# autonomousvision/gaussian-opacity-fields

Hardware: NVIDIA H100
Metric: training views/sec (fwd+bwd) @1080p, 1M Gaussians (higher is better)
Workload: dtype f32

## Files before the change

### gaussian-opacity-fields_b200/csrc/api.cu

```cuda
#include <stdarg.h>
#include <stdlib.h>

#include <chrono>

#include "gof_common.cuh"

static bool gof_trace_on() {
  static int on = -1;
  if (on < 0) { const char* e = getenv("GOF_TRACE"); on = (e && e[0] == '1') ? 1 : 0; }
  return on == 1;
}
struct GofTrace {
  std::chrono::steady_clock::time_point t0 = std::chrono::steady_clock::now();
  double last = 0;
  void mark(const char* what) {
    if (!gof_trace_on()) return;
    double t = std::chrono::duration<double, std::micro>(std::chrono::steady_clock::now() - t0).count();
    fprintf(stderr, "[gof trace] %-22s +%9.1f us (t=%9.1f us)\n", what, t - last, t);
    last = t;
  }
};

#include <map>
#include <mutex>
// ... 106 lines not shown
  static thread_local SideCopy table[64];
  int dev = 0;
  if (cudaGetDevice(&dev) != cudaSuccess || dev < 0 || dev >= 64) return nullptr;
  SideCopy& s = table[dev];
  if (!s.tried) {
    s.tried = true;
    s.ok = cudaStreamCreateWithFlags(&s.st, cudaStreamNonBlocking) == cudaSuccess &&
           cudaEventCreateWithFlags(&s.after_kernel, cudaEventDisableTiming) == cudaSuccess &&
           cudaEventCreateWithFlags(&s.copied, cudaEventDisableTiming) == cudaSuccess &&
           cudaHostAlloc((void**)&s.pin, 64, cudaHostAllocDefault) == cudaSuccess;
    if (!s.ok) (void)cudaGetLastError();
  }
  return s.ok ? &s : nullptr;
}
}

static SideCopy* begin_async_read_u32(const void* src_dev, cudaStream_t st) {
  SideCopy* sc = side_copy_for_current_device();
  if (!sc) return nullptr;
  if (cudaEventRecord(sc->after_kernel, st) != cudaSuccess || cudaStreamWaitEvent(sc->st, sc->after_kernel, 0) != cudaSuccess ||
      cudaMemcpyAsync(sc->pin, src_dev, 4, cudaMemcpyDeviceToHost, sc->st) != cudaSuccess ||
      cudaEventRecord(sc->copied, sc->st) != cudaSuccess) {
    (void)cudaGetLastError();
    return nullptr;
  }
  return sc;
}
static int finish_async_read_u32(SideCopy* sc, uint32_t* out) {
  GOF_CUDA_OK(cudaEventSynchronize(sc->copied));
  *out = *sc->pin;
  return GOF_OK;
}

static int preprocess_sort_count(const gof_scene_t* s, const GofView& v, char* geom, const GofGeomLayout& GL, int* radii,
                                 float box_margin, cudaStream_t st, uint32_t* R) {
  int rc;
  if ((rc = gof_launch_preprocess(s, v, geom, GL, radii, box_margin, st)) != GOF_OK) return rc;
  SideCopy* sc = s->debug ? nullptr : begin_async_read_u32(geom + GL.total, st);
  if ((rc = gof_depth_sort(s->P, geom, GL, s->debug != 0, st)) != GOF_OK) return rc;
  if (sc) return finish_async_read_u32(sc, R);
  return gof_read_back(R, geom + GL.total, sizeof(uint32_t), st);
}

static unsigned long long* g_stats_dev = nullptr;
unsigned long long* gof_stats_buffer() {
  static int on = -1;
  if (on < 0) { const char* e = getenv("GOF_STATS"); on = (e && e[0] == '1') ? 1 : 0; }
  if (!on) return nullptr;
  if (!g_stats_dev) { cudaMalloc(&g_stats_dev, 8 * sizeof(unsigned long long)); cudaMemset(g_stats_dev, 0, 8 * sizeof(unsigned long long)); }
  return g_stats_dev;
}
extern "C" int gof_stats_read(unsigned long long* out) {
  if (!gof_stats_buffer()) return 0;
  cudaMemcpy(out, g_stats_dev, 8 * sizeof(unsigned long long), cudaMemcpyDeviceToHost);
  cudaMemset(g_stats_dev, 0, 8 * sizeof(unsigned long long));
  return 1;
}

static thread_local char g_err[1024] = "";

void gof_set_error(const char* fmt, ...) {
  va_list ap;
  va_start(ap, fmt);
  vsnprintf(g_err, sizeof(g_err), fmt, ap);
  va_end(ap);
}

extern "C" const char* gof_last_error(void) { return g_err; }
extern "C" int gof_version(void) { return 100; }

// ... 25 lines not shown
  if (!has_sr && !s->view2gaussian_precomp) {
    gof_set_error("scales/rotations absent: view2gaussian_precomp is required");
    return GOF_E_INVALID;
  }
  if (s->width > 16 * 65535 || s->height > 16 * 65535) { gof_set_error("image too large"); return GOF_E_INVALID; }
  return GOF_OK;
}

extern "C" int gof_rasterize_forward(const gof_scene_t* s, gof_alloc_fn geom_alloc, void* geom_user,
                                     gof_alloc_fn binning_alloc, void* binning_user, gof_alloc_fn image_alloc,
                                     void* image_user, float* out_color, int* radii, int* num_rendered,
                                     void* stream) {
  int rc = validate_scene(s);
  if (rc != GOF_OK) return rc;
  if (!geom_alloc || !binning_alloc || !image_alloc || !num_rendered) {
    gof_set_error("allocators / num_rendered must be non-NULL");
    return GOF_E_INVALID;
  }
  *num_rendered = 0;
  cudaStream_t st = (cudaStream_t)stream;
  if (s->P == 0) return GOF_OK;
  if (!out_color || !radii) { gof_set_error("out_color / radii must be non-NULL"); return GOF_E_INVALID; }
  const GofView v = gof_make_view(s);

  GofTrace tr;
  const GofGeomLayout GL = gof_geom_layout((size_t)s->P);
  char* geom = (char*)geom_alloc(geom_user, GL.bytes);
  const GofImageLayout IL = gof_image_layout(s->width, s->height);
  char* img = (char*)image_alloc(image_user, IL.bytes);
  if (!geom || !img) { gof_set_error("scratch allocator returned NULL"); return GOF_E_ALLOC; }
  tr.mark("alloc geom+img");

  uint32_t R = 0;
  if ((rc = preprocess_sort_count(s, v, geom, GL, radii, 0.0f, st, &R)) != GOF_OK) return rc;
  *num_rendered = (int)R;
  tr.mark("pre+sort, num_rendered");

  const GofBinLayout BL = gof_bin_layout((size_t)R, s->width, s->height);
  char* bin = (char*)binning_alloc(binning_user, BL.bytes);
  if (!bin && BL.bytes) { gof_set_error("binning allocator returned NULL"); return GOF_E_ALLOC; }
  tr.mark("alloc binning");

  if ((rc = gof_bin_tiles(s->P, (size_t)R, v, geom, GL, bin, BL, img, IL, s->debug != 0, st)) != GOF_OK) return rc;
  if ((rc = gof_launch_render_forward(s, v, geom, GL, bin, BL, img, IL, out_color, st)) != GOF_OK) return rc;
  tr.mark("launch bin+render");
  return GOF_OK;
}

extern "C" int gof_rasterize_backward(const gof_scene_t* s, int num_rendered, const int* radii,
                                      void* geom_buffer, const void* binning_buffer,
                                      const void* image_buffer, const float* dL_dpix, float* dL_dmean2D,
                                      float* dL_dconic, float* dL_dopacity, float* dL_dcolor, float* dL_dmean3D,
                                      float* dL_dcov3D, float* dL_dsh, float* dL_dscale, float* dL_drot,
                                      float* dL_dview2gaussian, void* stream) {
  return gof_rasterize_backward_stats(s, num_rendered, radii, geom_buffer, binning_buffer, image_buffer, dL_dpix, dL_dmean2D, dL_dconic,
                                      dL_dopacity, dL_dcolor, dL_dmean3D, dL_dcov3D, dL_dsh, dL_dscale, dL_drot, dL_dview2gaussian,
                                      nullptr, nullptr, stream);
}

extern "C" int gof_rasterize_backward_stats(const gof_scene_t* s, int num_rendered, const int* radii, void* geom_buffer,
                                            const void* binning_buffer, const void* image_buffer, const float* dL_dpix,
                                            float* dL_dmean2D, float* dL_dconic, float* dL_dopacity, float* dL_dcolor,
                                            float* dL_dmean3D, float* dL_dcov3D, float* dL_dsh, float* dL_dscale, float* dL_drot,
                                            float* dL_dview2gaussian, float* dens_sum, float* dens_max, void* stream) {
  return gof_rasterize_backward_dp(s, num_rendered, radii, geom_buffer, binning_buffer, image_buffer, dL_dpix, dL_dmean2D, dL_dconic,
                                   dL_dopacity, dL_dcolor, dL_dmean3D, dL_dcov3D, dL_dsh, dL_dscale, dL_drot, dL_dview2gaussian, dens_sum,
                                   dens_max, nullptr, nullptr, stream);
// ... 247 lines not shown
```

### gaussian-opacity-fields_b200/csrc/binning.cu

```cuda
#include "gof_common.cuh"

namespace {

constexpr int THREADS = GOF_BLOCK_SIZE;
constexpr int WARPS = THREADS / 32;
constexpr uint32_t LB_AGG = 1u << 30;
constexpr uint32_t LB_INC = 2u << 30;
constexpr uint32_t LB_VAL = (1u << 30) - 1u;
constexpr size_t LB_MAX_ITEMS = (size_t)1 << 30;

__device__ __forceinline__ uint32_t ld_volatile(const uint32_t* p) { return *reinterpret_cast<const volatile uint32_t*>(p); }
__device__ __forceinline__ void st_volatile(uint32_t* p, uint32_t v) { *reinterpret_cast<volatile uint32_t*>(p) = v; }
__device__ __forceinline__ uint64_t ld_volatile(const uint64_t* p) { return *reinterpret_cast<const volatile uint64_t*>(p); }
__device__ __forceinline__ void st_volatile(uint64_t* p, uint64_t v) { *reinterpret_cast<volatile uint64_t*>(p) = v; }

template <typename W> struct LbWord;
template <> struct LbWord<uint32_t> {
  static constexpr int SHIFT = 30;
  static constexpr uint32_t VAL = LB_VAL;
};
template <> struct LbWord<uint64_t> {
  static constexpr int SHIFT = 32;
  static constexpr uint64_t VAL = 0xffffffffull;
};
// ... 35 lines not shown
}
__device__ __forceinline__ uint32_t lookback_digit_walk(uint32_t* status, uint32_t digit, uint32_t chunk, uint32_t aggregate) {
  uint32_t* own = status + ((size_t)(chunk >> 2) * GOF_RADIX + digit) * 4 + (chunk & 3u);
  if (chunk == 0) return 0u;
  uint32_t excl = 0u;
  uint32_t pos = chunk;
  while (pos > 0) {
    const uint32_t g = (pos - 1u) >> 2;
    const uint32_t need = pos - 4u * g;
    const uint32_t* word = status + ((size_t)g * GOF_RADIX + digit) * 4;
    uint4 w;
    bool ready;
    do {
      w = ld_volatile_v4(word);
      ready = (w.x >> 30) != 0u && (need < 2u || (w.y >> 30) != 0u) && (need < 3u || (w.z >> 30) != 0u) && (need < 4u || (w.w >> 30) != 0u);
    } while (!ready);
    const uint32_t e[4] = {w.x, w.y, w.z, w.w};
    bool done = false;
#pragma unroll
    for (int i = 3; i >= 0; --i) {
      if (!done && (uint32_t)i < need) {
        excl += e[i] & LB_VAL;
        if ((e[i] >> 30) == 2u) done = true;
      }
    }
    if (done) break;
    pos = 4u * g;
  }
  st_volatile(own, LB_INC | (excl + aggregate));
  return excl;
}

struct Digits { int shift[4]; uint32_t mask[4]; int passes; };

template <typename KeyT>
__global__ void __launch_bounds__(THREADS) k_digit_hist(const KeyT* __restrict__ keys, size_t n, Digits dg, uint32_t* __restrict__ ghist) {
  __shared__ uint32_t s_h[4][GOF_RADIX];
#pragma unroll
  for (int p = 0; p < 4; ++p) s_h[p][threadIdx.x] = 0;
  __syncthreads();
  const size_t stride = (size_t)gridDim.x * THREADS;
  for (size_t i = (size_t)blockIdx.x * THREADS + threadIdx.x; i < n; i += stride) {
    const uint32_t k = (uint32_t)keys[i];
#pragma unroll
    for (int p = 0; p < 4; ++p)
      if (p < dg.passes) atomicAdd(&s_h[p][(k >> dg.shift[p]) & dg.mask[p]], 1u);
  }
  __syncthreads();
#pragma unroll
  for (int p = 0; p < 4; ++p)
    if (p < dg.passes && s_h[p][threadIdx.x]) atomicAdd(ghist + p * GOF_RADIX + threadIdx.x, s_h[p][threadIdx.x]);
}

template <typename KeyT>
__global__ void __launch_bounds__(THREADS, 3) k_onesweep(const KeyT* __restrict__ keys_in, const uint32_t* __restrict__ vals_in,
                                                        KeyT* __restrict__ keys_out, uint32_t* __restrict__ vals_out, size_t n,
                                                        int shift, uint32_t mask, const uint32_t* __restrict__ ghist,
                                                        uint32_t* __restrict__ status ,
                                                        uint32_t* __restrict__ ticket) {
  __shared__ uint32_t s_cnt[WARPS][GOF_RADIX];
  __shared__ uint32_t s_gbase[GOF_RADIX];
  __shared__ uint32_t s_lbase[GOF_RADIX];
  __shared__ KeyT s_keys[GOF_SORT_CHUNK];
  __shared__ uint32_t s_vals[GOF_SORT_CHUNK];
  __shared__ uint32_t s_chunk;
  const int lane = threadIdx.x & 31, warp = threadIdx.x >> 5;
  if (threadIdx.x == 0) s_chunk = atomicAdd(ticket, 1u);
#pragma unroll
  for (int w = 0; w < WARPS; ++w) s_cnt[w][threadIdx.x] = 0;
  uint32_t dig_total;
  const uint32_t gstart = block_excl_scan(threadIdx.x <= mask ? ghist[threadIdx.x] : 0u, &dig_total);
  const uint32_t chunk = s_chunk;
  const size_t cbase = (size_t)chunk * GOF_SORT_CHUNK;
  const size_t wbase = cbase + (size_t)warp * (GOF_SORT_ITEMS * 32);

  KeyT key[GOF_SORT_ITEMS];
  uint32_t rank[GOF_SORT_ITEMS];
#pragma unroll
  for (int r = 0; r < GOF_SORT_ITEMS; ++r) {
    const size_t i = wbase + (size_t)r * 32 + lane;
    key[r] = i < n ? keys_in[i] : (KeyT)0;
  }
  const uint32_t lt = (1u << lane) - 1u;
#pragma unroll
  for (int r = 0; r < GOF_SORT_ITEMS; ++r) {
    const size_t i = wbase + (size_t)r * 32 + lane;
    const bool valid = i < n;
    const uint32_t d = valid ? (((uint32_t)key[r] >> shift) & mask) : (uint32_t)GOF_RADIX;
    const uint32_t peers = __match_any_sync(0xffffffffu, d);
    const int leader = __ffs(peers) - 1;
    uint32_t old = 0;
    if (lane == leader && valid) {
      old = s_cnt[warp][d];
      s_cnt[warp][d] = old + __popc(peers);
    }
    old = __shfl_sync(0xffffffffu, old, leader);
    rank[r] = old + __popc(peers & lt);
    __syncwarp();
  }
  __syncthreads();
  uint32_t count = 0;
  if (threadIdx.x <= mask) {
#pragma unroll
    for (int w = 0; w < WARPS; ++w) {
      const uint32_t c = s_cnt[w][threadIdx.x];
      s_cnt[w][threadIdx.x] = count;
      count += c;
    }
    lookback_digit_publish(status, threadIdx.x, chunk, count);
  }
  uint32_t chunk_n;
  const uint32_t lstart = block_excl_scan(count, &chunk_n);
  s_lbase[threadIdx.x] = lstart;
  __syncthreads();
#pragma unroll
  for (int r = 0; r < GOF_SORT_ITEMS; ++r) {
    const size_t i = wbase + (size_t)r * 32 + lane;
    if (i < n) {
      const uint32_t d = ((uint32_t)key[r] >> shift) & mask;
      const uint32_t lp = s_lbase[d] + s_cnt[warp][d] + rank[r];
      s_keys[lp] = key[r];
      s_vals[lp] = vals_in[i];
    }
  }
  if (threadIdx.x <= mask) s_gbase[threadIdx.x] = gstart + lookback_digit_walk(status, threadIdx.x, chunk, count);
  __syncthreads();
#pragma unroll
  for (int r = 0; r < GOF_SORT_ITEMS; ++r) {
    const uint32_t i = (uint32_t)r * THREADS + threadIdx.x;
    if (i < chunk_n) {
      const KeyT k = s_keys[i];
      const uint32_t d = ((uint32_t)k >> shift) & mask;
      const uint32_t pos = s_gbase[d] + (i - s_lbase[d]);
      keys_out[pos] = k;
      vals_out[pos] = s_vals[i];
    }
  }
}

struct SortScratch {
  uint32_t* ghist;
  uint32_t* tickets;
  uint32_t* status;
  size_t pass_words;
};

SortScratch carve_sort_scratch(uint32_t* scratch, size_t n) {
  SortScratch s;
  s.ghist = scratch;
  s.tickets = scratch + 4 * GOF_RADIX;
  s.status = scratch + GOF_SORT_HEAD_BYTES / 4;
  s.pass_words = (size_t)((gof_sort_blocks(n) + 3) / 4 + 1) * GOF_RADIX * 4;
  return s;
}

void split_digits(int nbits, Digits* dg) {
  dg->passes = (nbits + 7) / 8;
  int rem = nbits, shift = 0;
  for (int p = 0; p < 4; ++p) { dg->shift[p] = 0; dg->mask[p] = 0; }
  for (int p = 0; p < dg->passes; ++p) {
    const int b = (rem + (dg->passes - p) - 1) / (dg->passes - p);
    dg->shift[p] = shift; dg->mask[p] = (1u << b) - 1u;
    shift += b; rem -= b;
  }
}

template <typename KeyT>
int onesweep_passes(KeyT* ka, KeyT* kb, uint32_t* va, uint32_t* vb, size_t n, const Digits& dg, const SortScratch& sc, bool debug,
                    cudaStream_t st) {
  const unsigned nb = (unsigned)gof_sort_blocks(n);
  for (int p = 0; p < dg.passes; ++p) {
    const bool a2b = (p % 2 == 0);
    GOF_LAUNCH("radix_onesweep", st, (k_onesweep<KeyT><<<nb, THREADS, 0, st>>>(
        a2b ? ka : kb, a2b ? va : vb, a2b ? kb : ka, a2b ? vb : va, n, dg.shift[p], dg.mask[p], sc.ghist + p * GOF_RADIX,
        sc.status + (size_t)p * sc.pass_words, sc.tickets + p)));
    GOF_LAUNCH_CHECK(debug, st);
  }
  return GOF_OK;
}

int sm_count() {
  static int sms = 0;
  if (!sms) { int dev = 0; cudaGetDevice(&dev); cudaDeviceGetAttribute(&sms, cudaDevAttrMultiProcessorCount, dev); if (sms <= 0) sms = 132; }
  return sms;
}

template <typename KeyT>
int sort_pairs(KeyT* ka, KeyT* kb, uint32_t* va, uint32_t* vb, uint32_t* scratch, size_t n, int nbits, bool debug, cudaStream_t st,
               int* result_in_b) {
  *result_in_b = 0;
  if (n == 0 || nbits <= 0) return GOF_OK;
  if (n >= LB_MAX_ITEMS) { gof_set_error("radix sort of %zu items: fewer than 2^30 supported", n); return GOF_E_INVALID; }
  Digits dg;
  split_digits(nbits, &dg);
  const SortScratch sc = carve_sort_scratch(scratch, n);
  GOF_CUDA_OK(cudaMemsetAsync(scratch, 0, GOF_SORT_HEAD_BYTES + (size_t)dg.passes * sc.pass_words * 4, st));
  const size_t want = (n + (size_t)THREADS * 8 - 1) / ((size_t)THREADS * 8);
  const unsigned grid = (unsigned)(want < (size_t)sm_count() * 4 ? want : (size_t)sm_count() * 4);
  GOF_LAUNCH("radix_hist", st, k_digit_hist<KeyT><<<grid, THREADS, 0, st>>>(ka, n, dg, sc.ghist));
  GOF_LAUNCH_CHECK(debug, st);
  const int rc = onesweep_passes<KeyT>(ka, kb, va, vb, n, dg, sc, debug, st);
  *result_in_b = dg.passes % 2;
  return rc;
}

__global__ void __launch_bounds__(THREADS) k_scan_excl(const uint32_t* __restrict__ in, uint32_t* __restrict__ out, size_t n,
                                                      uint64_t* __restrict__ status, uint32_t* __restrict__ ticket,
                                                      uint32_t* __restrict__ total_out, uint32_t nchunks) {
  __shared__ uint32_t s_chunk, s_prefix;
  if (threadIdx.x == 0) s_chunk = atomicAdd(ticket, 1u);
  __syncthreads();
  const uint32_t chunk = s_chunk;
  const size_t base = (size_t)chunk * GOF_SCAN_CHUNK + (size_t)threadIdx.x * GOF_SCAN_ITEMS;
  uint32_t v[GOF_SCAN_ITEMS];
  uint32_t s = 0;
#pragma unroll
  for (int k = 0; k < GOF_SCAN_ITEMS; ++k) {
    v[k] = (base + k < n) ? in[base + k] : 0u;
    s += v[k];
  }
  uint32_t total;
  uint32_t run = block_excl_scan(s, &total);
  if (threadIdx.x < 32) {
    const uint32_t excl = lookback_warp(status, chunk, total);
    if (threadIdx.x == 0) {
      s_prefix = excl;
      if (chunk == nchunks - 1 && total_out) *total_out = excl + total;
    }
  }
  __syncthreads();
  run += s_prefix;
#pragma unroll
  for (int k = 0; k < GOF_SCAN_ITEMS; ++k) {
    if (base + k < n) out[base + k] = run;
    run += v[k];
  }
}

template <typename KeyT>
__global__ void __launch_bounds__(THREADS) k_scan_emit(int P, const uint32_t* __restrict__ order, const uint2* __restrict__ rect,
                                                      const uint32_t* __restrict__ tiles, int grid_x, KeyT* __restrict__ keys,
                                                      uint32_t* __restrict__ vals, uint32_t* __restrict__ status,
                                                      uint32_t* __restrict__ ticket, Digits dg, uint32_t* __restrict__ ghist,
                                                      uint32_t capacity) {
  __shared__ uint32_t s_off[THREADS + 1];
  __shared__ uint32_t s_g[THREADS];
  __shared__ uint2 s_rect[THREADS];
  __shared__ uint32_t s_h[2][GOF_RADIX];
  __shared__ uint32_t s_chunk, s_prefix;
  if (threadIdx.x == 0) s_chunk = atomicAdd(ticket, 1u);
  s_h[0][threadIdx.x] = 0; s_h[1][threadIdx.x] = 0;
  __syncthreads();
  const uint32_t chunk = s_chunk;
  const int k = (int)(chunk * THREADS + threadIdx.x);
  uint32_t g = 0, n = 0;
  uint2 rc = make_uint2(0u, 0u);
  if (k < P) {
    g = order[k];
    n = tiles[g];
    if (n) rc = rect[g];
  }
  uint32_t total;
  const uint32_t lo = block_excl_scan(n, &total);
  s_off[threadIdx.x] = lo; s_g[threadIdx.x] = g; s_rect[threadIdx.x] = rc;
  if (threadIdx.x < 32) {
    const uint32_t excl = lookback_warp(status, chunk, total);
    if (threadIdx.x == 0) { s_off[THREADS] = total; s_prefix = excl; }
  }
  __syncthreads();
  const uint32_t prefix = s_prefix;
  for (uint32_t j = threadIdx.x; j < total; j += THREADS) {
    int lo_i = 0, hi_i = THREADS;
    while (hi_i - lo_i > 1) {
      const int mid = (lo_i + hi_i) >> 1;
      if (s_off[mid] <= j) lo_i = mid; else hi_i = mid;
    }
    const uint32_t t = j - s_off[lo_i];
    const uint2 r = s_rect[lo_i];
    const uint32_t xmin = r.x & 0xffffu, ymin = r.x >> 16;
    const uint32_t w = (r.y & 0xffffu) - xmin;
    const uint32_t dy = t / w, dx = t - dy * w;
    const uint32_t tile = (ymin + dy) * (uint32_t)grid_x + xmin + dx;
    const uint32_t pos = prefix + j;
    if (pos < capacity) {
      keys[pos] = (KeyT)tile;
      vals[pos] = s_g[lo_i];
    }
    atomicAdd(&s_h[0][(tile >> dg.shift[0]) & dg.mask[0]], 1u);
    if (dg.passes > 1) atomicAdd(&s_h[1][(tile >> dg.shift[1]) & dg.mask[1]], 1u);
  }
// ... 16 lines not shown
      ranges[cur].x = (uint32_t)idx;
    }
  }
  if (idx == L - 1) ranges[cur].y = (uint32_t)L;
}

template <typename KeyT>
int bin_tiles_t(int P, size_t R, const GofView& v, char* geom, const GofGeomLayout& GL, char* bin, const GofBinLayout& BL, char* img,
                const GofImageLayout& IL, bool debug, cudaStream_t st) {
  if (R >= LB_MAX_ITEMS) { gof_set_error("binning: %zu (tile, Gaussian) instances, fewer than 2^30 supported", R); return GOF_E_INVALID; }
  uint2* ranges = reinterpret_cast<uint2*>(img + IL.ranges);
  GOF_CUDA_OK(cudaMemsetAsync(ranges, 0, (size_t)v.tiles * sizeof(uint2), st));
  if (R == 0) return GOF_OK;
  KeyT* ka = reinterpret_cast<KeyT*>(bin + BL.key_a);
  KeyT* kb = reinterpret_cast<KeyT*>(bin + BL.key_b);
  uint32_t* va = reinterpret_cast<uint32_t*>(bin + BL.val_a);
  uint32_t* vb = reinterpret_cast<uint32_t*>(bin + BL.val_b);
  uint32_t* scratch = reinterpret_cast<uint32_t*>(bin + BL.hist);
  Digits dg;
  dg.passes = BL.passes;
  int shift = 0;
  for (int p = 0; p < 4; ++p) {
    dg.shift[p] = shift; dg.mask[p] = p < BL.passes ? (1u << BL.bits[p]) - 1u : 0u;
    shift += BL.bits[p];
  }
  if (BL.passes > 2) { gof_set_error("tile ids need more than two radix digits"); return GOF_E_INVALID; }
  const SortScratch sc = carve_sort_scratch(scratch, R);
  GOF_CUDA_OK(cudaMemsetAsync(scratch, 0, GOF_SORT_HEAD_BYTES + (size_t)dg.passes * sc.pass_words * 4, st));
  uint32_t* scan_status = reinterpret_cast<uint32_t*>(geom + GL.scan_tmp);
  const int nchunks = (P + THREADS - 1) / THREADS;
  GOF_CUDA_OK(cudaMemsetAsync(scan_status, 0, ((size_t)nchunks + 8) * 4, st));
  const uint32_t* order = reinterpret_cast<const uint32_t*>(geom + GL.val_a);
  GOF_LAUNCH("scan_emit", st, k_scan_emit<KeyT><<<nchunks, THREADS, 0, st>>>(
      P, order, reinterpret_cast<const uint2*>(geom + GL.rect), reinterpret_cast<const uint32_t*>(geom + GL.tiles), v.grid_x, ka, va,
      scan_status, scan_status + nchunks + 4, dg, sc.ghist, (uint32_t)R));
  GOF_LAUNCH_CHECK(debug, st);
  const int rc = onesweep_passes<KeyT>(ka, kb, va, vb, R, dg, sc, debug, st);
  if (rc != GOF_OK) return rc;
  const KeyT* sorted = reinterpret_cast<const KeyT*>(bin + BL.sorted_keys);
  GOF_LAUNCH("tile_ranges", st, k_tile_ranges<KeyT><<<(unsigned)((R + 255) / 256), 256, 0, st>>>(R, sorted, ranges, 0));
  GOF_LAUNCH_CHECK(debug, st);
  return GOF_OK;
}


__global__ void __launch_bounds__(THREADS) k_sort_init(size_t n, const uint32_t* __restrict__ w0, uint32_t* __restrict__ ka,
                                                      uint32_t* __restrict__ vals) {
  const size_t i = (size_t)blockIdx.x * THREADS + threadIdx.x;
  if (i >= n) return;
  vals[i] = (uint32_t)i;
  if (w0) ka[i] = w0[i];
}

__global__ void __launch_bounds__(THREADS) k_gather_word(size_t n, const uint32_t* __restrict__ word, const uint32_t* __restrict__ ord,
                                                        uint32_t* __restrict__ keys) {
  const size_t j = (size_t)blockIdx.x * THREADS + threadIdx.x;
  if (j < n) keys[j] = word[ord[j]];
}

__global__ void __launch_bounds__(THREADS) k_run_heads(size_t n, const GofKeyWords key, const uint32_t* __restrict__ ord,
                                                      uint32_t* __restrict__ head) {
  const size_t j = (size_t)blockIdx.x * THREADS + threadIdx.x;
  if (j >= n) return;
  if (j == 0) { head[0] = 1; return; }
  const uint32_t a = ord[j], b = ord[j - 1];
  uint32_t diff = 0;
#pragma unroll
  for (int k = 0; k < 3; ++k) {
    if (k >= key.nw) break;
    const uint32_t mask = key.bits[k] >= 32 ? 0xffffffffu : (1u << key.bits[k]) - 1u;
    diff |= (key.w[k][a] ^ key.w[k][b]) & mask;
  }
  head[j] = diff ? 1u : 0u;
}

}

int gof_depth_sort(int P, char* geom, const GofGeomLayout& L, bool debug, cudaStream_t st) {
  int in_b = 0;
  return sort_pairs<uint32_t>(reinterpret_cast<uint32_t*>(geom + L.key_a), reinterpret_cast<uint32_t*>(geom + L.key_b),
                              reinterpret_cast<uint32_t*>(geom + L.val_a), reinterpret_cast<uint32_t*>(geom + L.val_b),
                              reinterpret_cast<uint32_t*>(geom + L.hist), (size_t)P, 32, debug, st, &in_b);
}

int gof_sort_points_by_tile(size_t n, int nbits, int key_shift, uint32_t* ka, uint32_t* kb, uint32_t* va, uint32_t* vb, uint32_t* hist,
                            uint2* ranges, int num_tiles, bool debug, cudaStream_t st, int* result_in_b) {
  GOF_CUDA_OK(cudaMemsetAsync(ranges, 0, (size_t)(num_tiles + 1) * sizeof(uint2), st));
  *result_in_b = 0;
  if (n == 0) return GOF_OK;
  const int rc = sort_pairs<uint32_t>(ka, kb, va, vb, hist, n, nbits, debug, st, result_in_b);
  if (rc != GOF_OK) return rc;
  const uint32_t* sorted = *result_in_b ? kb : ka;
  GOF_LAUNCH("tile_ranges", st, k_tile_ranges<uint32_t><<<(unsigned)((n + 255) / 256), 256, 0, st>>>(n, sorted, ranges, key_shift));
  GOF_LAUNCH_CHECK(debug, st);
  return GOF_OK;
}

int gof_exclusive_scan_u32(const uint32_t* in, uint32_t* out, uint32_t* tmp, uint32_t* total, size_t n, bool debug, cudaStream_t st) {
  if (n == 0) {
    if (total) GOF_CUDA_OK(cudaMemsetAsync(total, 0, 4, st));
    return GOF_OK;
  }
  if (reinterpret_cast<uintptr_t>(tmp) % 8u) { gof_set_error("exclusive_scan: tmp must be 8-byte aligned"); return GOF_E_INVALID; }
  const uint32_t nchunks = (uint32_t)((n + GOF_SCAN_CHUNK - 1) / GOF_SCAN_CHUNK);
  GOF_CUDA_OK(cudaMemsetAsync(tmp, 0, ((size_t)nchunks * 2 + 1) * 4, st));
  GOF_LAUNCH("scan", st, k_scan_excl<<<nchunks, THREADS, 0, st>>>(in, out, n, reinterpret_cast<uint64_t*>(tmp), tmp + (size_t)nchunks * 2,
                                                                  total, nchunks));
  GOF_LAUNCH_CHECK(debug, st);
  return GOF_OK;
}

int gof_sort_words_u32(const GofKeyWords& key, size_t n, const GofSortBufs& b, uint32_t* ord, bool debug, cudaStream_t st) {
  if (key.nw < 1 || key.nw > 3 || (ord != b.va && ord != b.vb)) { gof_set_error("sort_words: 1-3 words, ord = va or vb"); return GOF_E_INVALID; }
  int passes = 0;
  for (int k = 0; k < key.nw; ++k) {
    if (key.bits[k] < 1 || key.bits[k] > 32) { gof_set_error("sort_words: %d bits in word %d", key.bits[k], k); return GOF_E_INVALID; }
    passes += (key.bits[k] + 7) / 8;
  }
  if (n == 0) return GOF_OK;
  if (n >= LB_MAX_ITEMS) { gof_set_error("sort_words: %zu items, the radix sort takes fewer than 2^30", n); return GOF_E_INVALID; }
  uint32_t* vals = passes % 2 == 0 ? ord : (ord == b.va ? b.vb : b.va);
  uint32_t* spare = vals == b.va ? b.vb : b.va;
  const unsigned grid = (unsigned)((n + THREADS - 1) / THREADS);
  GOF_LAUNCH("sort_init", st, k_sort_init<<<grid, THREADS, 0, st>>>(n, key.w[0] == b.ka ? nullptr : key.w[0], b.ka, vals));
  GOF_LAUNCH_CHECK(debug, st);
  for (int k = 0; k < key.nw; ++k) {
    if (k > 0) {
      GOF_LAUNCH("sort_gather", st, k_gather_word<<<grid, THREADS, 0, st>>>(n, key.w[k], vals, b.ka));
      GOF_LAUNCH_CHECK(debug, st);
    }
    int in_b = 0;
    const int rc = sort_pairs<uint32_t>(b.ka, b.kb, vals, spare, b.hist, n, key.bits[k], debug, st, &in_b);
    if (rc != GOF_OK) return rc;
    if (in_b) { uint32_t* t = vals; vals = spare; spare = t; }
  }
  return GOF_OK;
}

int gof_key_runs_u32(const GofKeyWords& key, const uint32_t* ord, size_t n, uint32_t* head, uint32_t* run, uint32_t* scan_tmp,
                     uint32_t* num_runs, bool debug, cudaStream_t st) {
  if (key.nw < 1 || key.nw > 3) { gof_set_error("key_runs: 1-3 words"); return GOF_E_INVALID; }
  if (n > 0) {
    GOF_LAUNCH("run_heads", st, k_run_heads<<<(unsigned)((n + THREADS - 1) / THREADS), THREADS, 0, st>>>(n, key, ord, head));
    GOF_LAUNCH_CHECK(debug, st);
  }
  return gof_exclusive_scan_u32(head, run, scan_tmp, num_runs, n, debug, st);
}

int gof_bin_tiles(int P, size_t R, const GofView& v, char* geom, const GofGeomLayout& GL, char* bin, const GofBinLayout& BL,
                  char* img, const GofImageLayout& IL, bool debug, cudaStream_t st) {
  if (BL.key_bytes == 2) return bin_tiles_t<uint16_t>(P, R, v, geom, GL, bin, BL, img, IL, debug, st);
  return bin_tiles_t<uint32_t>(P, R, v, geom, GL, bin, BL, img, IL, debug, st);
}

namespace {
GofKeyWords probe_key(int nw, const uint32_t* const* words, const int* bits) {
  GofKeyWords key{};
  key.nw = nw;
  for (int k = 0; k < nw && k < 3; ++k) { key.w[k] = words[k]; key.bits[k] = bits[k]; }
  return key;
}
}

extern "C" GOF_API int gof_probe_sort_words_u32(int nw, const uint32_t* const* words, const int* bits, size_t n, uint32_t* ka,
                                                uint32_t* kb, uint32_t* va, uint32_t* vb, uint32_t* hist, int ord_is_vb, void* stream) {
// ... 18 lines not shown
```

### gaussian-opacity-fields_b200/csrc/gof_common.cuh

```cuda
#pragma once
#include <cuda_runtime.h>
#include <stdint.h>
#include <stdio.h>
#include <string.h>

#include "../../include/gof_rasterizer.h"

#define GOF_BLOCK_X 16
#define GOF_BLOCK_Y 16
#define GOF_BLOCK_SIZE 256

void gof_set_error(const char* fmt, ...);

#define GOF_CUDA_OK(expr)                                                                      \
  do {                                                                                         \
    cudaError_t _e = (expr);                                                                   \
    if (_e != cudaSuccess) {                                                                   \
      gof_set_error("%s:%d: %s -> %s", __FILE__, __LINE__, #expr, cudaGetErrorString(_e));     \
      return GOF_E_CUDA;                                                                       \
    }                                                                                          \
  } while (0)

#define GOF_LAUNCH_CHECK(debug, stream)                                                        \
  do {                                                                                         \
// ... 130 lines not shown

struct __align__(16) GofSplatBwd {
  float mx, my;
  float cx, cy, cz;
  uint32_t self;
  float pad[2];
};
static_assert(sizeof(GofSplatBwd) == 32, "GofSplatBwd must be 32 bytes");

static inline size_t gof_align_up(size_t v, size_t a) { return (v + a - 1) / a * a; }

#define GOF_SORT_ITEMS 16
#define GOF_SORT_CHUNK (GOF_BLOCK_SIZE * GOF_SORT_ITEMS)
#define GOF_RADIX 256

static constexpr inline int gof_sort_blocks(size_t n) { return (int)((n + GOF_SORT_CHUNK - 1) / GOF_SORT_CHUNK); }

#define GOF_SORT_HEAD_BYTES (4 * GOF_RADIX * 4 + 256)
static constexpr inline size_t gof_sort_scratch_bytes(size_t n) {
  return (size_t)GOF_SORT_HEAD_BYTES + (size_t)4 * ((size_t)gof_sort_blocks(n) + 8) * GOF_RADIX * 4;
}

#define GOF_SCAN_ITEMS 8
#define GOF_SCAN_CHUNK (GOF_BLOCK_SIZE * GOF_SCAN_ITEMS)

static constexpr inline size_t gof_scan_scratch_bytes(size_t n) { return (n / GOF_SCAN_CHUNK + 4) * 8 + 4096; }

struct GofGeomLayout {
  size_t splat, splat_bwd, rect, tiles, clamped, depth;
  size_t key_a, key_b, val_a, val_b;
  size_t hist;
  size_t scan_tmp;
  size_t total;
  size_t grad_acc;
  size_t reject_k;
  size_t bytes;
};

static inline GofGeomLayout gof_geom_layout(size_t P) {
  GofGeomLayout L;
  size_t o = 0;
  auto take = [&](size_t bytes) { size_t r = o; o = gof_align_up(o + bytes, 256); return r; };
  L.splat = take(P * sizeof(GofSplat));
  L.splat_bwd = take(P * sizeof(GofSplatBwd));
  L.rect = take(P * 8);
  L.tiles = take(P * 4);
  L.clamped = take(P);
  L.depth = take(P * 4);
  L.key_a = take(P * 4);
  L.key_b = take(P * 4);
  L.val_a = take(P * 4);
  L.val_b = take(P * 4);
  L.hist = take(gof_sort_scratch_bytes(P));
  L.scan_tmp = take((P / 256 + 8) * 4 + 4096);
  L.total = take(256);
  L.grad_acc = take(P * 128);
  L.reject_k = take(P * 4);
  L.bytes = o;
  return L;
}

struct GofImageLayout {
  size_t accum;
  size_t ncontrib;
  size_t ranges;
  size_t bytes;
};

static inline GofImageLayout gof_image_layout(int W, int H) {
  const size_t tiles = (size_t)((W + 15) / 16) * ((H + 15) / 16);
  GofImageLayout L;
  size_t o = 0;
  auto take = [&](size_t bytes) { size_t r = o; o = gof_align_up(o + bytes, 256); return r; };
  L.accum = take(tiles * 256 * 4 * 4);
  L.ncontrib = take(tiles * 256 * 2 * 4);
  L.ranges = take(tiles * 8);
  L.bytes = o;
  return L;
}

struct GofBinLayout {
  size_t key_a, key_b;
  size_t val_a, val_b;
  size_t hist;
  int key_bytes;
  int passes;
  int bits[4];
  size_t point_list;
// ... 84 lines not shown
  GofPointLayout L; size_t o = 0;
  auto take = [&](size_t b) { size_t r = o; o = gof_align_up(o + b, 256); return r; };
  L.xy = take(PN * 8); L.depth = take(PN * 4); L.bytes = o; return L;
}
#define GOF_INT_MAX_CONTRIB 1024
static inline GofPointBinLayout gof_point_bin_layout(size_t PN, int tiles, int sm_count) {
  GofPointBinLayout L; size_t o = 0;
  auto take = [&](size_t b) { size_t r = o; o = gof_align_up(o + b, 256); return r; };
  L.key_a = take(PN * 4); L.key_b = take(PN * 4); L.val_a = take(PN * 4); L.val_b = take(PN * 4);
  L.hist = take(gof_sort_scratch_bytes(PN));
  L.pranges = take((size_t)(tiles + 1) * 8);
  L.nblk = tiles < sm_count * 3 ? tiles : sm_count * 3;
  if (L.nblk < 1) L.nblk = 1;
  L.ids = take((size_t)L.nblk * 256 * GOF_INT_MAX_CONTRIB * 2);
  L.bytes = o; return L;
}
int gof_launch_integrate(const gof_scene_t* s, const GofView& v, int PN, const float* points3D, const GofSplat* splat,
                         const uint32_t* point_list, const uint2* ranges, char* img, const GofImageLayout& IL, char* pts,
                         const GofPointLayout& PL, char* pbin, const GofPointBinLayout& PBL, float* out_color, float* out_alpha,
                         float* out_color_int, cudaStream_t st);

struct GofIntCacheLayout { size_t splat, ranges, point_list, bytes; };
static inline GofIntCacheLayout gof_int_cache_layout(size_t P, int W, int H, size_t R) {
  const size_t tiles = (size_t)((W + 15) / 16) * ((H + 15) / 16);
  GofIntCacheLayout L; size_t o = 0;
  auto take = [&](size_t b) { size_t r = o; o = gof_align_up(o + b, 256); return r; };
  L.splat = take(P * sizeof(GofSplat)); L.ranges = take(tiles * 8); L.point_list = take(R * 4); L.bytes = o;
  return L;
}

int gof_launch_render_forward(const gof_scene_t* s, const GofView& v, const char* geom,
                              const GofGeomLayout& GL, char* bin, const GofBinLayout& BL, char* img,
                              const GofImageLayout& IL, float* out_color, cudaStream_t st);
int gof_launch_render_backward(const gof_scene_t* s, const GofView& v, char* geom,
                               const GofGeomLayout& GL, const char* bin, const GofBinLayout& BL,
                               const char* img, const GofImageLayout& IL, const float* dL_dpix, cudaStream_t st);
```

### gaussian-opacity-fields_b200/csrc/render_bwd.cu

```cuda
#include "gof_common.cuh"
#include "gof_math.cuh"

namespace {

struct BwdArgs {
  int W, H, grid_x;
  float focal_x, focal_y;
  const uint2* ranges;
  const uint32_t* point_list;
  const GofSplat* splat;
  const GofSplatBwd* splat_bwd;
  const float* bg;
  const float* accum;
  const uint32_t* ncontrib;
  const float* dL_dpix;
  size_t plane;
  const uint32_t* vmask;
  size_t vstride;
  double* grad_acc;
  unsigned long long* stats;
};

constexpr int BATCH = GOF_BLOCK_SIZE;
constexpr int GROUPS = BATCH / 32;
// ... 196 lines not shown
      first = (uint32_t)hb * 8u;
      qb = quarter_word(s_quarter + first);
      mybits = s_mask[first + lane];
    };
    next_group();
    while (__any_sync(0xffffffffu, qb != 0u)) {
      const bool act = qb != 0u;
      const int b = act ? 31 - __clz(qb) : 0;
      if (act) qb &= ~(1u << b);
      const uint32_t row = s_base + (first + (uint32_t)b) * 96u;
      const bool contrib = act && ((mybits >> b) & 1u) != 0u;
      if (STATS) { st_visit += (lane == 0); st_anyhit += act && !(lane & 11); }
      float g[16];
      pair_grad(row, (uint32_t)base + first + (uint32_t)b, contrib, g);
      float r0, r1;
      quarter_reduce16(g, lane, &r0, &r1);
      if (act) {
        const uint32_t gid = __float_as_uint(gof_lds32<84>(row));
        double* dst = a.grad_acc + ((size_t)gid * 16 + ((lane & 8) ? 1 : 0) + ((lane & 2) ? 2 : 0) + ((lane & 1) ? 4 : 0));
        if (r0 != 0.f) atomicAdd(dst, (double)r0);
        if (r1 != 0.f) atomicAdd(dst + 8, (double)r1);
        if (STATS) st_red += (r0 != 0.f) + (r1 != 0.f);
      }
      if (qb == 0u) next_group();
    }
  }
  if (STATS && a.stats) {
    atomicAdd(a.stats + 0, st_visit); atomicAdd(a.stats + 1, st_eval); atomicAdd(a.stats + 2, st_pass);
    atomicAdd(a.stats + 3, st_contrib); atomicAdd(a.stats + 4, st_anyhit); atomicAdd(a.stats + 7, st_red);
    if (threadIdx.x == 0) { atomicAdd(a.stats + 5, (unsigned long long)used); atomicAdd(a.stats + 6, (unsigned long long)(range.y - range.x)); }
  }
}

template <bool STATS>
int launch_backward(const BwdArgs& a, int tiles, cudaStream_t st) {
  static bool attr_set = false;
  if (!attr_set) {
    const int need = (STATS ? 3 : 4) * (SMEM_BYTES + 1024);
    GOF_CUDA_OK(cudaFuncSetAttribute(k_render_backward<STATS>, cudaFuncAttributePreferredSharedMemoryCarveout,
                                     (need * 100 + 233471) / 233472 > 100 ? 100 : (need * 100 + 233471) / 233472));
    attr_set = true;
  }
  GOF_LAUNCH("render_bwd", st, k_render_backward<STATS><<<tiles, GOF_BLOCK_SIZE, SMEM_BYTES, st>>>(a));
  return GOF_OK;
}

}

int gof_launch_render_backward(const gof_scene_t* s, const GofView& v, char* geom, const GofGeomLayout& GL,
                               const char* bin, const GofBinLayout& BL, const char* img, const GofImageLayout& IL,
                               const float* dL_dpix, cudaStream_t st) {
  BwdArgs a{};
  a.W = v.W; a.H = v.H; a.grid_x = v.grid_x; a.focal_x = v.focal_x; a.focal_y = v.focal_y;
  a.ranges = reinterpret_cast<const uint2*>(img + IL.ranges);
  a.point_list = reinterpret_cast<const uint32_t*>(bin + BL.point_list);
  a.splat = reinterpret_cast<const GofSplat*>(geom + GL.splat);
  a.splat_bwd = reinterpret_cast<const GofSplatBwd*>(geom + GL.splat_bwd);
  a.bg = s->background;
  a.accum = reinterpret_cast<const float*>(img + IL.accum);
  a.ncontrib = reinterpret_cast<const uint32_t*>(img + IL.ncontrib);
  a.dL_dpix = dL_dpix;
  a.plane = (size_t)v.tiles * 256;
  a.vmask = reinterpret_cast<const uint32_t*>(bin + BL.vmask);
  a.vstride = BL.vmask_stride;
  a.grad_acc = reinterpret_cast<double*>(geom + GL.grad_acc);
  GOF_CUDA_OK(cudaMemsetAsync(a.grad_acc, 0, (size_t)s->P * 128, st));
  a.stats = gof_stats_buffer();
  const int rc = a.stats ? launch_backward<true>(a, v.tiles, st) : launch_backward<false>(a, v.tiles, st);
  if (rc != GOF_OK) return rc;
  GOF_LAUNCH_CHECK(s->debug, st);
  return GOF_OK;
}
```

Baseline: 249.7.

## Overlap grad accumulator clear with forward sort and drop culled keys from depth sort

```diff
diff --git a/gaussian-opacity-fields_b200/csrc/api.cu b/gaussian-opacity-fields_b200/csrc/api.cu
--- a/gaussian-opacity-fields_b200/csrc/api.cu
+++ b/gaussian-opacity-fields_b200/csrc/api.cu
@@ -162,10 +162,34 @@
   return GOF_OK;
 }
 
+namespace {
+struct SideClear { cudaStream_t st = nullptr; cudaEvent_t fork = nullptr, join = nullptr; bool ok = false, tried = false; };
+SideClear* side_clear_for_current_device() {
+  static thread_local SideClear table[64];
+  int dev = 0;
+  if (cudaGetDevice(&dev) != cudaSuccess || dev < 0 || dev >= 64) return nullptr;
+  SideClear& s = table[dev];
+  if (!s.tried) {
+    s.tried = true;
+    s.ok = cudaStreamCreateWithFlags(&s.st, cudaStreamNonBlocking) == cudaSuccess &&
+           cudaEventCreateWithFlags(&s.fork, cudaEventDisableTiming) == cudaSuccess &&
+           cudaEventCreateWithFlags(&s.join, cudaEventDisableTiming) == cudaSuccess;
+    if (!s.ok) (void)cudaGetLastError();
+  }
+  return s.ok ? &s : nullptr;
+}
+}
+
 static int preprocess_sort_count(const gof_scene_t* s, const GofView& v, char* geom, const GofGeomLayout& GL, int* radii,
-                                 float box_margin, cudaStream_t st, uint32_t* R) {
+                                 float box_margin, cudaStream_t st, uint32_t* R, SideClear* clear = nullptr) {
   int rc;
   if ((rc = gof_launch_preprocess(s, v, geom, GL, radii, box_margin, st)) != GOF_OK) return rc;
+  if (clear) {
+    GOF_CUDA_OK(cudaEventRecord(clear->fork, st));
+    GOF_CUDA_OK(cudaStreamWaitEvent(clear->st, clear->fork, 0));
+    if ((rc = gof_launch_clear_acc(s->P, geom, GL, clear->st)) != GOF_OK) return rc;
+    GOF_CUDA_OK(cudaEventRecord(clear->join, clear->st));
+  }
   SideCopy* sc = s->debug ? nullptr : begin_async_read_u32(geom + GL.total, st);
   if ((rc = gof_depth_sort(s->P, geom, GL, s->debug != 0, st)) != GOF_OK) return rc;
   if (sc) return finish_async_read_u32(sc, R);
@@ -257,7 +281,13 @@
   tr.mark("alloc geom+img");
 
   uint32_t R = 0;
-  if ((rc = preprocess_sort_count(s, v, geom, GL, radii, 0.0f, st, &R)) != GOF_OK) return rc;
+  SideClear* clear = side_clear_for_current_device();
+  if (!clear && (rc = gof_launch_clear_acc(s->P, geom, GL, st)) != GOF_OK) return rc;
+  struct Join {
+    SideClear* c; cudaStream_t st;
+    ~Join() { if (c) (void)cudaStreamWaitEvent(st, c->join, 0); }
+  } join{clear, st};
+  if ((rc = preprocess_sort_count(s, v, geom, GL, radii, 0.0f, st, &R, clear)) != GOF_OK) return rc;
   *num_rendered = (int)R;
   tr.mark("pre+sort, num_rendered");
 
diff --git a/gaussian-opacity-fields_b200/csrc/binning.cu b/gaussian-opacity-fields_b200/csrc/binning.cu
--- a/gaussian-opacity-fields_b200/csrc/binning.cu
+++ b/gaussian-opacity-fields_b200/csrc/binning.cu
@@ -91,9 +91,11 @@
 }
 
 struct Digits { int shift[4]; uint32_t mask[4]; int passes; };
+constexpr uint32_t DROP_KEY = 0xffffffffu;
 
 template <typename KeyT>
-__global__ void __launch_bounds__(THREADS) k_digit_hist(const KeyT* __restrict__ keys, size_t n, Digits dg, uint32_t* __restrict__ ghist) {
+__global__ void __launch_bounds__(THREADS) k_digit_hist(const KeyT* __restrict__ keys, size_t n, Digits dg, bool drop,
+                                                       uint32_t* __restrict__ ghist) {
   __shared__ uint32_t s_h[4][GOF_RADIX];
 #pragma unroll
   for (int p = 0; p < 4; ++p) s_h[p][threadIdx.x] = 0;
@@ -101,6 +103,7 @@
   const size_t stride = (size_t)gridDim.x * THREADS;
   for (size_t i = (size_t)blockIdx.x * THREADS + threadIdx.x; i < n; i += stride) {
     const uint32_t k = (uint32_t)keys[i];
+    if (drop && k == DROP_KEY) continue;
 #pragma unroll
     for (int p = 0; p < 4; ++p)
       if (p < dg.passes) atomicAdd(&s_h[p][(k >> dg.shift[p]) & dg.mask[p]], 1u);
@@ -111,7 +114,7 @@
     if (p < dg.passes && s_h[p][threadIdx.x]) atomicAdd(ghist + p * GOF_RADIX + threadIdx.x, s_h[p][threadIdx.x]);
 }
 
-template <typename KeyT>
+template <typename KeyT, bool DROP>
 __global__ void __launch_bounds__(THREADS, 3) k_onesweep(const KeyT* __restrict__ keys_in, const uint32_t* __restrict__ vals_in,
                                                         KeyT* __restrict__ keys_out, uint32_t* __restrict__ vals_out, size_t n,
                                                         int shift, uint32_t mask, const uint32_t* __restrict__ ghist,
@@ -129,8 +132,10 @@
   for (int w = 0; w < WARPS; ++w) s_cnt[w][threadIdx.x] = 0;
   uint32_t dig_total;
   const uint32_t gstart = block_excl_scan(threadIdx.x <= mask ? ghist[threadIdx.x] : 0u, &dig_total);
+  if (!DROP) n = dig_total;
   const uint32_t chunk = s_chunk;
   const size_t cbase = (size_t)chunk * GOF_SORT_CHUNK;
+  if (cbase >= n) return;
   const size_t wbase = cbase + (size_t)warp * (GOF_SORT_ITEMS * 32);
 
   KeyT key[GOF_SORT_ITEMS];
@@ -144,7 +149,7 @@
 #pragma unroll
   for (int r = 0; r < GOF_SORT_ITEMS; ++r) {
     const size_t i = wbase + (size_t)r * 32 + lane;
-    const bool valid = i < n;
+    const bool valid = i < n && !(DROP && (uint32_t)key[r] == DROP_KEY);
     const uint32_t d = valid ? (((uint32_t)key[r] >> shift) & mask) : (uint32_t)GOF_RADIX;
     const uint32_t peers = __match_any_sync(0xffffffffu, d);
     const int leader = __ffs(peers) - 1;
@@ -175,7 +180,7 @@
 #pragma unroll
   for (int r = 0; r < GOF_SORT_ITEMS; ++r) {
     const size_t i = wbase + (size_t)r * 32 + lane;
-    if (i < n) {
+    if (i < n && !(DROP && (uint32_t)key[r] == DROP_KEY)) {
       const uint32_t d = ((uint32_t)key[r] >> shift) & mask;
       const uint32_t lp = s_lbase[d] + s_cnt[warp][d] + rank[r];
       s_keys[lp] = key[r];
@@ -225,12 +230,13 @@
 }
 
 template <typename KeyT>
-int onesweep_passes(KeyT* ka, KeyT* kb, uint32_t* va, uint32_t* vb, size_t n, const Digits& dg, const SortScratch& sc, bool debug,
-                    cudaStream_t st) {
+int onesweep_passes(KeyT* ka, KeyT* kb, uint32_t* va, uint32_t* vb, size_t n, const Digits& dg, bool drop, const SortScratch& sc,
+                    bool debug, cudaStream_t st) {
   const unsigned nb = (unsigned)gof_sort_blocks(n);
   for (int p = 0; p < dg.passes; ++p) {
     const bool a2b = (p % 2 == 0);
-    GOF_LAUNCH("radix_onesweep", st, (k_onesweep<KeyT><<<nb, THREADS, 0, st>>>(
+    auto* kernel = drop && p == 0 ? k_onesweep<KeyT, true> : k_onesweep<KeyT, false>;
+    GOF_LAUNCH("radix_onesweep", st, (kernel<<<nb, THREADS, 0, st>>>(
         a2b ? ka : kb, a2b ? va : vb, a2b ? kb : ka, a2b ? vb : va, n, dg.shift[p], dg.mask[p], sc.ghist + p * GOF_RADIX,
         sc.status + (size_t)p * sc.pass_words, sc.tickets + p)));
     GOF_LAUNCH_CHECK(debug, st);
@@ -245,8 +251,8 @@
 }
 
 template <typename KeyT>
-int sort_pairs(KeyT* ka, KeyT* kb, uint32_t* va, uint32_t* vb, uint32_t* scratch, size_t n, int nbits, bool debug, cudaStream_t st,
-               int* result_in_b) {
+int sort_pairs(KeyT* ka, KeyT* kb, uint32_t* va, uint32_t* vb, uint32_t* scratch, size_t n, int nbits, bool drop, bool debug,
+               cudaStream_t st, int* result_in_b) {
   *result_in_b = 0;
   if (n == 0 || nbits <= 0) return GOF_OK;
   if (n >= LB_MAX_ITEMS) { gof_set_error("radix sort of %zu items: fewer than 2^30 supported", n); return GOF_E_INVALID; }
@@ -256,9 +262,9 @@
   GOF_CUDA_OK(cudaMemsetAsync(scratch, 0, GOF_SORT_HEAD_BYTES + (size_t)dg.passes * sc.pass_words * 4, st));
   const size_t want = (n + (size_t)THREADS * 8 - 1) / ((size_t)THREADS * 8);
   const unsigned grid = (unsigned)(want < (size_t)sm_count() * 4 ? want : (size_t)sm_count() * 4);
-  GOF_LAUNCH("radix_hist", st, k_digit_hist<KeyT><<<grid, THREADS, 0, st>>>(ka, n, dg, sc.ghist));
+  GOF_LAUNCH("radix_hist", st, k_digit_hist<KeyT><<<grid, THREADS, 0, st>>>(ka, n, dg, drop, sc.ghist));
   GOF_LAUNCH_CHECK(debug, st);
-  const int rc = onesweep_passes<KeyT>(ka, kb, va, vb, n, dg, sc, debug, st);
+  const int rc = onesweep_passes<KeyT>(ka, kb, va, vb, n, dg, drop, sc, debug, st);
   *result_in_b = dg.passes % 2;
   return rc;
 }
@@ -297,9 +303,9 @@
 }
 
 template <typename KeyT>
-__global__ void __launch_bounds__(THREADS) k_scan_emit(int P, const uint32_t* __restrict__ order, const uint2* __restrict__ rect,
-                                                      const uint32_t* __restrict__ tiles, int grid_x, KeyT* __restrict__ keys,
-                                                      uint32_t* __restrict__ vals, uint32_t* __restrict__ status,
+__global__ void __launch_bounds__(THREADS) k_scan_emit(const uint32_t* __restrict__ depth_hist, const uint32_t* __restrict__ order,
+                                                      const uint2* __restrict__ rect, const uint32_t* __restrict__ tiles, int grid_x,
+                                                      KeyT* __restrict__ keys, uint32_t* __restrict__ vals, uint32_t* __restrict__ status,
                                                       uint32_t* __restrict__ ticket, Digits dg, uint32_t* __restrict__ ghist,
                                                       uint32_t capacity) {
   __shared__ uint32_t s_off[THREADS + 1];
@@ -309,12 +315,14 @@
   __shared__ uint32_t s_chunk, s_prefix;
   if (threadIdx.x == 0) s_chunk = atomicAdd(ticket, 1u);
   s_h[0][threadIdx.x] = 0; s_h[1][threadIdx.x] = 0;
-  __syncthreads();
+  uint32_t V;
+  block_excl_scan(depth_hist[threadIdx.x], &V);
   const uint32_t chunk = s_chunk;
-  const int k = (int)(chunk * THREADS + threadIdx.x);
+  if (chunk * THREADS >= V) return;
+  const uint32_t k = chunk * THREADS + threadIdx.x;
   uint32_t g = 0, n = 0;
   uint2 rc = make_uint2(0u, 0u);
-  if (k < P) {
+  if (k < V) {
     g = order[k];
     n = tiles[g];
     if (n) rc = rect[g];
@@ -397,10 +405,11 @@
   GOF_CUDA_OK(cudaMemsetAsync(scan_status, 0, ((size_t)nchunks + 8) * 4, st));
   const uint32_t* order = reinterpret_cast<const uint32_t*>(geom + GL.val_a);
   GOF_LAUNCH("scan_emit", st, k_scan_emit<KeyT><<<nchunks, THREADS, 0, st>>>(
-      P, order, reinterpret_cast<const uint2*>(geom + GL.rect), reinterpret_cast<const uint32_t*>(geom + GL.tiles), v.grid_x, ka, va,
-      scan_status, scan_status + nchunks + 4, dg, sc.ghist, (uint32_t)R));
+      reinterpret_cast<const uint32_t*>(geom + GL.hist), order, reinterpret_cast<const uint2*>(geom + GL.rect),
+      reinterpret_cast<const uint32_t*>(geom + GL.tiles), v.grid_x, ka, va, scan_status, scan_status + nchunks + 4, dg, sc.ghist,
+      (uint32_t)R));
   GOF_LAUNCH_CHECK(debug, st);
-  const int rc = onesweep_passes<KeyT>(ka, kb, va, vb, R, dg, sc, debug, st);
+  const int rc = onesweep_passes<KeyT>(ka, kb, va, vb, R, dg, false, sc, debug, st);
   if (rc != GOF_OK) return rc;
   const KeyT* sorted = reinterpret_cast<const KeyT*>(bin + BL.sorted_keys);
   GOF_LAUNCH("tile_ranges", st, k_tile_ranges<KeyT><<<(unsigned)((R + 255) / 256), 256, 0, st>>>(R, sorted, ranges, 0));
@@ -445,7 +454,7 @@
   int in_b = 0;
   return sort_pairs<uint32_t>(reinterpret_cast<uint32_t*>(geom + L.key_a), reinterpret_cast<uint32_t*>(geom + L.key_b),
                               reinterpret_cast<uint32_t*>(geom + L.val_a), reinterpret_cast<uint32_t*>(geom + L.val_b),
-                              reinterpret_cast<uint32_t*>(geom + L.hist), (size_t)P, 32, debug, st, &in_b);
+                              reinterpret_cast<uint32_t*>(geom + L.hist), (size_t)P, 32, true, debug, st, &in_b);
 }
 
 int gof_sort_points_by_tile(size_t n, int nbits, int key_shift, uint32_t* ka, uint32_t* kb, uint32_t* va, uint32_t* vb, uint32_t* hist,
@@ -453,7 +462,7 @@
   GOF_CUDA_OK(cudaMemsetAsync(ranges, 0, (size_t)(num_tiles + 1) * sizeof(uint2), st));
   *result_in_b = 0;
   if (n == 0) return GOF_OK;
-  const int rc = sort_pairs<uint32_t>(ka, kb, va, vb, hist, n, nbits, debug, st, result_in_b);
+  const int rc = sort_pairs<uint32_t>(ka, kb, va, vb, hist, n, nbits, false, debug, st, result_in_b);
   if (rc != GOF_OK) return rc;
   const uint32_t* sorted = *result_in_b ? kb : ka;
   GOF_LAUNCH("tile_ranges", st, k_tile_ranges<uint32_t><<<(unsigned)((n + 255) / 256), 256, 0, st>>>(n, sorted, ranges, key_shift));
@@ -495,7 +504,7 @@
       GOF_LAUNCH_CHECK(debug, st);
     }
     int in_b = 0;
-    const int rc = sort_pairs<uint32_t>(b.ka, b.kb, vals, spare, b.hist, n, key.bits[k], debug, st, &in_b);
+    const int rc = sort_pairs<uint32_t>(b.ka, b.kb, vals, spare, b.hist, n, key.bits[k], false, debug, st, &in_b);
     if (rc != GOF_OK) return rc;
     if (in_b) { uint32_t* t = vals; vals = spare; spare = t; }
   }
diff --git a/gaussian-opacity-fields_b200/csrc/gof_common.cuh b/gaussian-opacity-fields_b200/csrc/gof_common.cuh
--- a/gaussian-opacity-fields_b200/csrc/gof_common.cuh
+++ b/gaussian-opacity-fields_b200/csrc/gof_common.cuh
@@ -186,6 +186,7 @@
   size_t hist;
   size_t scan_tmp;
   size_t total;
+  size_t acc_dirty;
   size_t grad_acc;
   size_t reject_k;
   size_t bytes;
@@ -208,6 +209,7 @@
   L.hist = take(gof_sort_scratch_bytes(P));
   L.scan_tmp = take((P / 256 + 8) * 4 + 4096);
   L.total = take(256);
+  L.acc_dirty = L.total + 4;
   L.grad_acc = take(P * 128);
   L.reject_k = take(P * 4);
   L.bytes = o;
@@ -358,6 +360,7 @@
 int gof_launch_render_forward(const gof_scene_t* s, const GofView& v, const char* geom,
                               const GofGeomLayout& GL, char* bin, const GofBinLayout& BL, char* img,
                               const GofImageLayout& IL, float* out_color, cudaStream_t st);
+int gof_launch_clear_acc(int P, char* geom, const GofGeomLayout& GL, cudaStream_t st);
 int gof_launch_render_backward(const gof_scene_t* s, const GofView& v, char* geom,
                                const GofGeomLayout& GL, const char* bin, const GofBinLayout& BL,
                                const char* img, const GofImageLayout& IL, const float* dL_dpix, cudaStream_t st);
diff --git a/gaussian-opacity-fields_b200/csrc/render_bwd.cu b/gaussian-opacity-fields_b200/csrc/render_bwd.cu
--- a/gaussian-opacity-fields_b200/csrc/render_bwd.cu
+++ b/gaussian-opacity-fields_b200/csrc/render_bwd.cu
@@ -252,6 +252,18 @@
   }
 }
 
+__global__ void __launch_bounds__(256) k_clear_acc(uint4* __restrict__ rows, size_t n, const uint32_t* __restrict__ dirty) {
+  if (dirty && *dirty == 0u) return;
+  const uint4 z = make_uint4(0u, 0u, 0u, 0u);
+  for (size_t i = (size_t)blockIdx.x * blockDim.x + threadIdx.x; i < n; i += (size_t)gridDim.x * blockDim.x) rows[i] = z;
+}
+
+unsigned clear_grid() {
+  static int sms = 0;
+  if (!sms) { int dev = 0; cudaGetDevice(&dev); cudaDeviceGetAttribute(&sms, cudaDevAttrMultiProcessorCount, dev); if (sms <= 0) sms = 132; }
+  return (unsigned)sms;
+}
+
 template <bool STATS>
 int launch_backward(const BwdArgs& a, int tiles, cudaStream_t st) {
   static bool attr_set = false;
@@ -265,6 +277,13 @@
   return GOF_OK;
 }
 
+}
+
+int gof_launch_clear_acc(int P, char* geom, const GofGeomLayout& GL, cudaStream_t st) {
+  GOF_LAUNCH("acc_clear", st, k_clear_acc<<<clear_grid(), 256, 0, st>>>(reinterpret_cast<uint4*>(geom + GL.grad_acc), (size_t)P * 8,
+                                                                        nullptr));
+  GOF_CUDA_OK(cudaMemsetAsync(geom + GL.acc_dirty, 0, 4, st));
+  return GOF_OK;
 }
 
 int gof_launch_render_backward(const gof_scene_t* s, const GofView& v, char* geom, const GofGeomLayout& GL,
@@ -284,7 +303,9 @@
   a.vmask = reinterpret_cast<const uint32_t*>(bin + BL.vmask);
   a.vstride = BL.vmask_stride;
   a.grad_acc = reinterpret_cast<double*>(geom + GL.grad_acc);
-  GOF_CUDA_OK(cudaMemsetAsync(a.grad_acc, 0, (size_t)s->P * 128, st));
+  uint32_t* dirty = reinterpret_cast<uint32_t*>(geom + GL.acc_dirty);
+  GOF_LAUNCH("acc_clear", st, k_clear_acc<<<clear_grid(), 256, 0, st>>>(reinterpret_cast<uint4*>(a.grad_acc), (size_t)s->P * 8, dirty));
+  GOF_CUDA_OK(cudaMemsetAsync(dirty, 0xff, 4, st));
   a.stats = gof_stats_buffer();
   const int rc = a.stats ? launch_backward<true>(a, v.tiles, st) : launch_backward<false>(a, v.tiles, st);
   if (rc != GOF_OK) return rc;
```

Result: no change. 250.8 (median of 6 runs) (+0.5%).
